# lucidrains/audiolm-pytorch

Hardware: AMD Instinct MI355X
Metric: audio-tokens/sec fwd+bwd, CoarseTransformer d=1024 seq=2048 (higher is better)
Workload: dtype bf16

## Files before the change

### audiolm-pytorch_amd/csrc/gemm.hip

```cpp
#include <algorithm>
#include <cstdlib>
#include <type_traits>

#include "common.hpp"
#include "../../include/audiolm_hip.h"

#ifndef ALM_GEMM_AUX_A
#define ALM_GEMM_AUX_A 0
#endif
#ifndef ALM_GEMM_AUX_B
#define ALM_GEMM_AUX_B 0
#endif

namespace {

constexpr int BK = 64;
constexpr unsigned OOB = 0x80000000u;

typedef __attribute__((address_space(3))) void lds_void;

struct GemmParams {
    const bf16_t* A;
    const bf16_t* B;
    void* C;
// ... 60 lines not shown
                        if (OUT_F32) {
                            const int ch = c0 / 4;
                            *reinterpret_cast<float4*>(slab + lr * ROWB + ((ch ^ (lr & (NCH - 1))) << 4)) = make_float4(v[0], v[1], v[2], v[3]);
                        } else {
                            const int ch = c0 / 8;
                            *reinterpret_cast<uint2*>(slab + lr * ROWB + ((ch ^ (lr & (NCH - 1))) << 4) + lh * 8) =
                                make_uint2(pack_bf2(v[0], v[1]), pack_bf2(v[2], v[3]));
                        }
                    }
                constexpr int LPR = NCH;
                constexpr int RPI = 64 / LPR;
#pragma unroll
                for (int it = 0; it < 32 / RPI; ++it) {
                    const int row = it * RPI + lane / LPR, ch = lane % LPR;
                    const uint4 val = *reinterpret_cast<const uint4*>(slab + row * ROWB + ((ch ^ (row & (NCH - 1))) << 4));
                    const int gm = mrow0 + row, gn = ncol0 + ch * (16 / ES);
#if defined(ALM_GEMM_WHATIF_NOSTORE)
                    if (gm < p.M && gn < p.N && val.x == 0x7fc12345u) *reinterpret_cast<uint4*>(Cb + ((long long)gm * p.ldc + gn) * ES) = val;
#else
                    if (gm < p.M && gn < p.N) {
                        uint4* dst = reinterpret_cast<uint4*>(Cb + ((long long)gm * p.ldc + gn) * ES);
                        typedef unsigned int u32x4 __attribute__((ext_vector_type(4)));
                        if (p.nt_store) __builtin_nontemporal_store(u32x4{val.x, val.y, val.z, val.w}, reinterpret_cast<u32x4*>(dst)); else *dst = val;
                    }
#endif
                }
            }
            return;
        }
    }
    const long long coff = coff0;
    const bool vec_ok = OUT_F32 ? ((p.ldc & 3) == 0 && (coff & 3) == 0 && ((uintptr_t)p.C & 15) == 0)
                                : ((p.ldc & 3) == 0 && (coff & 3) == 0 && ((uintptr_t)p.C & 7) == 0);
#pragma unroll
    for (int i = 0; i < TM; ++i) {
        const int gm = m0 + wr * (BM / WM) + i * 32 + lr;
        if (gm >= p.M) continue;
#pragma unroll
        for (int j = 0; j < TNB; ++j) {
#pragma unroll
            for (int g = 0; g < 4; ++g) {
                const int gn = n0 + wc * (BN / WN) + j * 32 + 8 * g + 4 * lh;
                if (gn >= p.N) continue;
                float v[4];
#pragma unroll
                for (int c = 0; c < 4; ++c) {
                    v[c] = acc[i][j][4 * g + c] * p.alpha;
                    if (p.bias && gn + c < p.N) v[c] += p.bias[gn + c];
                }
                const long long idx = coff + (long long)gm * p.ldc + gn;
                if (OUT_F32) {
                    float* C = reinterpret_cast<float*>(p.C) + idx;
                    if (vec_ok && gn + 3 < p.N) {
                        float4 o = make_float4(v[0], v[1], v[2], v[3]);
                        if (p.accumulate) { const float4 w = *reinterpret_cast<const float4*>(C); o.x += w.x; o.y += w.y; o.z += w.z; o.w += w.w; }
                        *reinterpret_cast<float4*>(C) = o;
                    } else {
#pragma unroll
                        for (int c = 0; c < 4; ++c)
                            if (gn + c < p.N) C[c] = p.accumulate ? C[c] + v[c] : v[c];
                    }
                } else {
                    bf16_t* C = reinterpret_cast<bf16_t*>(p.C) + idx;
                    if (vec_ok && gn + 3 < p.N) {
                        if (p.accumulate) {
                            const uint2 w = *reinterpret_cast<const uint2*>(C);
                            v[0] += __uint_as_float(w.x << 16); v[1] += __uint_as_float(w.x & 0xffff0000u);
                            v[2] += __uint_as_float(w.y << 16); v[3] += __uint_as_float(w.y & 0xffff0000u);
                        }
                        *reinterpret_cast<uint2*>(C) = make_uint2(pack_bf2(v[0], v[1]), pack_bf2(v[2], v[3]));
                    } else {
#pragma unroll
                        for (int c = 0; c < 4; ++c)
                            if (gn + c < p.N) C[c] = f2bf(p.accumulate ? bf2f(C[c]) + v[c] : v[c]);
                    }
                }
            }
        }
    }
}

template <int N>
__device__ __forceinline__ void wait_vmcnt() {
    static_assert(N == 0 || N == 8 || N == 16, "add the literal");
    if constexpr (N == 0) asm volatile("s_waitcnt vmcnt(0)" ::: "memory");
    else if constexpr (N == 8) asm volatile("s_waitcnt vmcnt(8)" ::: "memory");
    else asm volatile("s_waitcnt vmcnt(16)" ::: "memory");
}

template <int BM, int BN, int WM, int WN, bool TNMODE, bool OUT_F32, int NS = 2>
__device__ __forceinline__ void gemm_body(const GemmParams& p, const int bx, const int by, const int bz) {
    extern __shared__ __attribute__((aligned(1024))) unsigned char smem[];
    constexpr int NW = WM * WN;
    constexpr int A_BYTES = BM * BK * 2, B_BYTES = BN * BK * 2, STAGE = A_BYTES + B_BYTES;
    constexpr int TM = BM / WM / 32, TNB = BN / WN / 32;
    constexpr int NIA = BM / 8 / NW, NIB = BN / 8 / NW;
    static_assert(NIA >= 1 && NIB >= 1 && (BM / 8) % NW == 0 && (BN / 8) % NW == 0, "tile / wave shape");

    const int tiles_m = (p.M + BM - 1) / BM, tiles_n = (p.N + BN - 1) / BN;
    int tm, tn, zb, zs;
    if (p.raster >= 1) {
        const int L = bx, xcd = L & 7, j = L >> 3;
        const bool m_major = tiles_m >= tiles_n;
        const int tmaj = m_major ? tiles_m : tiles_n, Q = m_major ? tiles_n : tiles_m;
        const int P = p.plimit > 0 ? p.plimit : tmaj * (p.nbt > 0 ? p.nbt : p.nb2);
        const int PL = (P + 7) / 8;
        zs = j / (PL * Q);
        const int rem = j % (PL * Q);
        const int panel = p.raster == 2 ? xcd * PL + rem / Q : (rem / Q) * 8 + xcd;
        const int minor = rem % Q;
        if (panel >= P || zs >= p.nsl) return;
        zb = panel / tmaj;
        const int tmajor = panel % tmaj;
        tm = m_major ? tmajor : minor;
        tn = m_major ? minor : tmajor;
    } else {
        const int nwg = tiles_m * tiles_n;
        const int bid = xcd_remap(bx, nwg);
        const int tt = grouped_tile(bid, tiles_m, tiles_n, p.group_m);
        tm = tt & 0xffff;
        tn = tt >> 16;
        zb = by;
        zs = bz;
    }
    const int m0 = tm * BM, n0 = tn * BN;

    const int z1 = zb / p.nb2, z2 = zb % p.nb2;
    int kbeg = 0, Krem = p.K;
    const long long zoffA = z1 * p.sA1 + z2 * p.sA2, zoffB = z1 * p.sB1 + z2 * p.sB2;
    if (p.ksplit > 0) {
        kbeg = zs * p.ksplit;
        Krem = min(p.K - kbeg, p.ksplit);
    }

    const int t = threadIdx.x;
    const int lane = t & 63;
    const int wave = __builtin_amdgcn_readfirstlane(t >> 6);
    const int wr = wave / WN, wc = wave % WN;
    const int lr = lane & 31, lh = lane >> 5;

    const bf16_t* Ab;
    const bf16_t* Bb;
    long long extA, extB;
    if (!TNMODE) {
        Ab = p.A + zoffA + (long long)m0 * p.lda + kbeg;
        Bb = p.B + zoffB + (long long)n0 * p.ldb + kbeg;
        extA = ((long long)(min(p.M - m0, BM) - 1) * p.lda + Krem) * 2;
        extB = ((long long)(min(p.N - n0, BN) - 1) * p.ldb + Krem) * 2;
    } else {
        Ab = p.A + zoffA + (long long)kbeg * p.lda + m0;
        Bb = p.B + zoffB + (long long)kbeg * p.ldb + n0;
        extA = ((long long)(Krem - 1) * p.lda + ((min(p.M - m0, BM) + 7) & ~7)) * 2;
        extB = ((long long)(Krem - 1) * p.ldb + ((min(p.N - n0, BN) + 7) & ~7)) * 2;
    }
    const auto rsA = __builtin_amdgcn_make_buffer_rsrc(const_cast<bf16_t*>(Ab), 0, (int)min(extA, 0x7fffffffLL), 0x00020000);
    const auto rsB = __builtin_amdgcn_make_buffer_rsrc(const_cast<bf16_t*>(Bb), 0, (int)min(extB, 0x7fffffffLL), 0x00020000);

    unsigned offA[NIA], offB[NIB];
    int kcA[NIA], kcB[NIB];
    if (!TNMODE) {
#pragma unroll
        for (int j = 0; j < NIA; ++j) {
            const int row = (j * NW + wave) * 8 + (lane >> 3);
            const int c = (lane & 7) ^ ((row >> 1) & 7);
            offA[j] = (unsigned)(row * p.lda * 2 + c * 16);
            kcA[j] = c * 8;
        }
#pragma unroll
// ... 367 lines not shown
    __builtin_amdgcn_s_barrier();

    if constexpr (INL) {
        typedef unsigned int u32x4 __attribute__((ext_vector_type(4)));
        constexpr int SLAB_BYTES = BM * BN * 4, NCHUNK = TM * TNB * 4;
        const int S = p.inl_slices;
        const int tile_lin = zb * (tiles_m * tiles_n) + tm * tiles_n + tn;
        unsigned char* const slab0 = reinterpret_cast<unsigned char*>(p.inl_ws) + (long long)tile_lin * S * SLAB_BYTES;
        {
            const auto rs = __builtin_amdgcn_make_buffer_rsrc(slab0 + (long long)zs * SLAB_BYTES, 0, SLAB_BYTES, 0x00020000);
#pragma unroll
            for (int i = 0; i < TM; ++i)
#pragma unroll
                for (int j = 0; j < TNB; ++j)
#pragma unroll
                    for (int g = 0; g < 4; ++g) {
                        const u32x4 v = {__float_as_uint(acc[i][j][4 * g]), __float_as_uint(acc[i][j][4 * g + 1]), __float_as_uint(acc[i][j][4 * g + 2]),
                                         __float_as_uint(acc[i][j][4 * g + 3])};
                        __builtin_amdgcn_raw_buffer_store_b128(v, rs, t * 16, ((i * TNB + j) * 4 + g) * 8192, 16);
                    }
        }
        asm volatile("s_waitcnt vmcnt(0)" ::: "memory");
        __syncthreads();
        unsigned* const flag = reinterpret_cast<unsigned*>(smem + 163840 - 16);
        if (t == 0) {
            const unsigned old = __hip_atomic_fetch_add(p.inl_cnt + tile_lin, 1u, __ATOMIC_RELAXED, __HIP_MEMORY_SCOPE_AGENT);
            const unsigned last = old == (unsigned)(S - 1);
            if (last) __hip_atomic_store(p.inl_cnt + tile_lin, 0u, __ATOMIC_RELAXED, __HIP_MEMORY_SCOPE_AGENT);
            *flag = last;
        }
        __syncthreads();
        if (*flag == 0) return;
        auto add_slab = [&](int sl, auto first_c) {
            constexpr bool FIRST = decltype(first_c)::value;
            const auto rs = __builtin_amdgcn_make_buffer_rsrc(slab0 + (long long)sl * SLAB_BYTES, 0, SLAB_BYTES, 0x00020000);
#pragma unroll
            for (int cb = 0; cb < NCHUNK; cb += 4) {
                u32x4 v[4];
#pragma unroll
                for (int c = 0; c < 4; ++c) v[c] = __builtin_amdgcn_raw_buffer_load_b128(rs, t * 16, (cb + c) * 8192, 16);
#pragma unroll
                for (int c = 0; c < 4; ++c)
#pragma unroll
                    for (int e = 0; e < 4; ++e) {
                        const int ai = (cb + c) / (4 * TNB), aj = ((cb + c) / 4) % TNB, ar = 4 * ((cb + c) % 4) + e;
                        acc[ai][aj][ar] = FIRST ? __uint_as_float(v[c][e]) : acc[ai][aj][ar] + __uint_as_float(v[c][e]);
                    }
            }
        };
        if (S == 2) {
            add_slab(1 - zs, std::false_type{});
        } else {
            add_slab(0, std::true_type{});
#pragma unroll 1
            for (int sl = 1; sl < S; ++sl) add_slab(sl, std::false_type{});
        }
    }

    const long long coff0 = z1 * p.sC1 + z2 * p.sC2 + (p.ksplit > 0 ? zs * p.sCk : 0);
    GPROBE_T(5);
    gemm_epilogue<BM, BN, WM, WN, TM, TNB, OUT_F32>(p, acc, smem, coff0, m0, n0, wave, wr, wc, lane, lr, lh);
    GPROBE_T(6);
    GPROBE_FLUSH((bx + gridDim.x * (by + gridDim.y * bz)) * 8 + wave);
}


template <bool TNMODE, bool OUT_F32>
__global__ __launch_bounds__(512) void gemm_stag_kernel(GemmParams p) {
    gemm_stag_body<TNMODE, OUT_F32>(p, blockIdx.x, blockIdx.y, blockIdx.z);
}

template <bool OUT_F32>
__global__ __launch_bounds__(512) void gemm_stag_inl_kernel(GemmParams p) {
    gemm_stag_body<false, OUT_F32, true>(p, blockIdx.x, blockIdx.y, blockIdx.z);
}

template <bool TNMODE, bool OUT_F32>
__global__ __launch_bounds__(512) void gemm_stag_group2_kernel(GemmParams p0, GemmParams p1, int tiles0) {
    const bool second = (int)blockIdx.x >= tiles0;
    const GemmParams& p = second ? p1 : p0;
    gemm_stag_body<TNMODE, OUT_F32>(p, second ? (int)blockIdx.x - tiles0 : (int)blockIdx.x, 0, 0);
}

template <bool TNMODE, bool OUT_F32>
__global__ __launch_bounds__(256) void gemm_w4_kernel(GemmParams p) {
    extern __shared__ __attribute__((aligned(1024))) unsigned char smem[];
    GPROBE_DECL
    constexpr int BM = 256, BN = 256, WM = 2, WN = 2, NW = 4, TM = 4, TNB = 4;
    constexpr int A_BYTES = BM * BK * 2, B_BYTES = BN * BK * 2, STAGE = A_BYTES + B_BYTES;
    constexpr int NIA = BM / 8 / NW, NIB = BN / 8 / NW;
    static_assert(NIA + NIB == 16, "the counted waits below assume 16 pieces per wave and stage");

    const int tiles_m = (p.M + BM - 1) / BM, tiles_n = (p.N + BN - 1) / BN;
    int tm, tn, zb, zs;
    if (p.raster >= 1) {
        const int L = blockIdx.x, xcd = L & 7, j = L >> 3;
        const bool m_major = tiles_m >= tiles_n;
        const int tmaj = m_major ? tiles_m : tiles_n, Q = m_major ? tiles_n : tiles_m;
        const int P = p.plimit > 0 ? p.plimit : tmaj * (p.nbt > 0 ? p.nbt : p.nb2);
        const int PL = (P + 7) / 8;
        zs = j / (PL * Q);
        const int rem = j % (PL * Q);
        const int panel = p.raster == 2 ? xcd * PL + rem / Q : (rem / Q) * 8 + xcd;
        const int minor = rem % Q;
        if (panel >= P || zs >= p.nsl) return;
        zb = panel / tmaj;
        const int tmajor = panel % tmaj;
        tm = m_major ? tmajor : minor;
        tn = m_major ? minor : tmajor;
    } else {
        const int nwg = tiles_m * tiles_n;
        const int bid = xcd_remap(blockIdx.x, nwg);
        const int tt = grouped_tile(bid, tiles_m, tiles_n, p.group_m);
        tm = tt & 0xffff;
        tn = tt >> 16;
        zb = blockIdx.y;
        zs = blockIdx.z;
    }
    const int m0 = tm * BM, n0 = tn * BN;
    const int z1 = zb / p.nb2, z2 = zb % p.nb2;
    int kbeg = 0, Krem = p.K;
    const long long zoffA = z1 * p.sA1 + z2 * p.sA2, zoffB = z1 * p.sB1 + z2 * p.sB2;
    if (p.ksplit > 0) {
        kbeg = zs * p.ksplit;
        Krem = min(p.K - kbeg, p.ksplit);
    }

    const int t = threadIdx.x;
    const int lane = t & 63;
    const int wave = __builtin_amdgcn_readfirstlane(t >> 6);
    const int wr = wave / WN, wc = wave % WN;
    const int lr = lane & 31, lh = lane >> 5;

    const bf16_t* Ab;
    const bf16_t* Bb;
    long long extA, extB;
    if (!TNMODE) {
        Ab = p.A + zoffA + (long long)m0 * p.lda + kbeg;
        Bb = p.B + zoffB + (long long)n0 * p.ldb + kbeg;
        extA = ((long long)(min(p.M - m0, BM) - 1) * p.lda + Krem) * 2;
        extB = ((long long)(min(p.N - n0, BN) - 1) * p.ldb + Krem) * 2;
    } else {
        Ab = p.A + zoffA + (long long)kbeg * p.lda + m0;
        Bb = p.B + zoffB + (long long)kbeg * p.ldb + n0;
        extA = ((long long)(Krem - 1) * p.lda + ((min(p.M - m0, BM) + 7) & ~7)) * 2;
        extB = ((long long)(Krem - 1) * p.ldb + ((min(p.N - n0, BN) + 7) & ~7)) * 2;
    }
    const auto rsA = __builtin_amdgcn_make_buffer_rsrc(const_cast<bf16_t*>(Ab), 0, (int)min(extA, 0x7fffffffLL), 0x00020000);
    const auto rsB = __builtin_amdgcn_make_buffer_rsrc(const_cast<bf16_t*>(Bb), 0, (int)min(extB, 0x7fffffffLL), 0x00020000);

    unsigned offA[NIA], offB[NIB];
    int kcA[NIA], kcB[NIB];
    if (!TNMODE) {
#pragma unroll
        for (int j = 0; j < NIA; ++j) {
            const int row = (j * NW + wave) * 8 + (lane >> 3);
            const int c = (lane & 7) ^ ((row >> 1) & 7);
            offA[j] = (unsigned)(row * p.lda * 2 + c * 16);
            kcA[j] = c * 8;
        }
#pragma unroll
        for (int j = 0; j < NIB; ++j) {
            const int row = (j * NW + wave) * 8 + (lane >> 3);
            const int c = (lane & 7) ^ ((row >> 1) & 7);
            offB[j] = (unsigned)(row * p.ldb * 2 + c * 16);
            kcB[j] = c * 8;
// ... 348 lines not shown
        }
        const uint4 pk = make_uint4(pack_bf2(e[0], e[1]), pack_bf2(e[2], e[3]), pack_bf2(e[4], e[5]), pack_bf2(e[6], e[7]));
        tile[i][cg * 4 + 0] = pk.x; tile[i][cg * 4 + 1] = pk.y; tile[i][cg * 4 + 2] = pk.z; tile[i][cg * 4 + 3] = pk.w;
        if (dst && r < q.rows_pad && c < q.cols_pad) *reinterpret_cast<uint4*>(dst + (long long)r * q.ld_dst + c) = pk;
    }
    if (!dstT) return;
    __syncthreads();
#pragma unroll
    for (int it = 0; it < 2; ++it) {
        const int w = it * 256 + t;
        const int rg = w & 7, cp = w >> 3;
        uint32_t a[8];
#pragma unroll
        for (int jj = 0; jj < 8; ++jj) a[jj] = tile[rg * 8 + jj][cp];
        const uint4 lo = make_uint4((a[0] & 0xffffu) | (a[1] << 16), (a[2] & 0xffffu) | (a[3] << 16), (a[4] & 0xffffu) | (a[5] << 16), (a[6] & 0xffffu) | (a[7] << 16));
        const uint4 hi = make_uint4((a[0] >> 16) | (a[1] & 0xffff0000u), (a[2] >> 16) | (a[3] & 0xffff0000u), (a[4] >> 16) | (a[5] & 0xffff0000u),
                                    (a[6] >> 16) | (a[7] & 0xffff0000u));
        const int oc = c0 + 2 * cp, orow = r0 + 8 * rg;
        if (orow < q.rows_pad) {
            if (oc < q.cols_pad) *reinterpret_cast<uint4*>(dstT + (long long)oc * q.ld_dstT + orow) = lo;
            if (oc + 1 < q.cols_pad) *reinterpret_cast<uint4*>(dstT + (long long)(oc + 1) * q.ld_dstT + orow) = hi;
        }
    }
}

template <int BM, int BN, int WM, int WN, bool TNMODE, bool OUT_F32>
int launch_cfg(const GemmParams& p, int ny, int nz, hipStream_t st) {
    constexpr int smem = 2 * (BM + BN) * BK * 2;
    static bool attr_done = false;
    auto kfn = gemm_kernel<BM, BN, WM, WN, TNMODE, OUT_F32>;
    if (!attr_done) {
        hipError_t e = hipFuncSetAttribute(reinterpret_cast<const void*>(kfn), hipFuncAttributeMaxDynamicSharedMemorySize, smem);
        if (e != hipSuccess) return (int)e;
        attr_done = true;
    }
    const int tiles_m = (p.M + BM - 1) / BM, tiles_n = (p.N + BN - 1) / BN;
    if (p.raster >= 1) {
        const int tmaj = tiles_m >= tiles_n ? tiles_m : tiles_n, Q = tiles_m >= tiles_n ? tiles_n : tiles_m;
        const int PL = ((p.plimit > 0 ? p.plimit : tmaj * ny) + 7) / 8;
        hipLaunchKernelGGL(kfn, dim3(8 * PL * Q * nz), dim3(WM * WN * 64), smem, st, p);
        return 0;
    }
    hipLaunchKernelGGL(kfn, dim3(tiles_m * tiles_n, ny, nz), dim3(WM * WN * 64), smem, st, p);
    return 0;
}

template <bool OUT_F32>
int launch_ring(const GemmParams& p, int ny, int nz, hipStream_t st) {
    constexpr int smem = 4 * (128 + 128) * BK * 2;
    static bool attr_done = false;
    auto kfn = gemm_ring_kernel<128, 128, 2, 2, false, OUT_F32, 4>;
    if (!attr_done) {
        hipError_t e = hipFuncSetAttribute(reinterpret_cast<const void*>(kfn), hipFuncAttributeMaxDynamicSharedMemorySize, smem);
        if (e != hipSuccess) return (int)e;
        attr_done = true;
    }
    hipLaunchKernelGGL(kfn, dim3(((p.M + 127) / 128) * ((p.N + 127) / 128), ny, nz), dim3(256), smem, st, p);
    return 0;
}

template <bool TNMODE, bool OUT_F32>
int launch_stag(const GemmParams& p, int ny, int nz, hipStream_t st) {
    constexpr int smem = 163840;
    static bool attr_done = false;
    auto kfn = gemm_stag_kernel<TNMODE, OUT_F32>;
    if (!attr_done) {
        hipError_t e = hipFuncSetAttribute(reinterpret_cast<const void*>(kfn), hipFuncAttributeMaxDynamicSharedMemorySize, smem);
        if (e != hipSuccess) return (int)e;
        attr_done = true;
    }
    const int tiles_m = (p.M + 255) / 256, tiles_n = (p.N + 255) / 256;
    if (p.raster >= 1) {
        const int tmaj = tiles_m >= tiles_n ? tiles_m : tiles_n, Q = tiles_m >= tiles_n ? tiles_n : tiles_m;
        const int PL = ((p.plimit > 0 ? p.plimit : tmaj * ny) + 7) / 8;
        hipLaunchKernelGGL(kfn, dim3(8 * PL * Q * nz), dim3(512), smem, st, p);
        return 0;
    }
    hipLaunchKernelGGL(kfn, dim3(tiles_m * tiles_n, ny, nz), dim3(512), smem, st, p);
    return 0;
}


template <bool OUT_F32>
int launch_stag_inl(const GemmParams& p, int ny, hipStream_t st) {
    constexpr int smem = 163840;
    static bool attr_done = false;
    auto kfn = gemm_stag_inl_kernel<OUT_F32>;
    if (!attr_done) {
        hipError_t e = hipFuncSetAttribute(reinterpret_cast<const void*>(kfn), hipFuncAttributeMaxDynamicSharedMemorySize, smem);
        if (e != hipSuccess) return (int)e;
        attr_done = true;
    }
    const int tiles_m = (p.M + 255) / 256, tiles_n = (p.N + 255) / 256;
    hipLaunchKernelGGL(kfn, dim3(tiles_m * tiles_n, ny, p.inl_slices), dim3(512), smem, st, p);
    return 0;
}

template <bool TNMODE, bool OUT_F32>
int launch_w4(const GemmParams& p, int ny, int nz, hipStream_t st) {
    constexpr int smem = 131072;
    static bool attr_done = false;
    auto kfn = gemm_w4_kernel<TNMODE, OUT_F32>;
    if (!attr_done) {
        hipError_t e = hipFuncSetAttribute(reinterpret_cast<const void*>(kfn), hipFuncAttributeMaxDynamicSharedMemorySize, smem);
        if (e != hipSuccess) return (int)e;
        attr_done = true;
    }
    const int tiles_m = (p.M + 255) / 256, tiles_n = (p.N + 255) / 256;
    if (p.raster >= 1) {
        const int tmaj = tiles_m >= tiles_n ? tiles_m : tiles_n, Q = tiles_m >= tiles_n ? tiles_n : tiles_m;
        const int PL = ((p.plimit > 0 ? p.plimit : tmaj * ny) + 7) / 8;
        hipLaunchKernelGGL(kfn, dim3(8 * PL * Q * nz), dim3(256), smem, st, p);
        return 0;
    }
    hipLaunchKernelGGL(kfn, dim3(tiles_m * tiles_n, ny, nz), dim3(256), smem, st, p);
    return 0;
}

int pick_tile(int M, int N, int ny, int tile, bool tn) {
    if (tile == 1 || tile == 2 || tile == 11 || tile == 13 || tile == 14 || tile == 15 || tile == 16 || tile == 17) return tile;
    if (tile != 0) return -1;
    if (M < 256 || N < 256) return 1;
    const long long t256 = (long long)((M + 255) / 256) * ((N + 255) / 256) * ny;
    if (t256 < 192) return 1;
    if (!tn) {
        static const double c320 = [] { const char* e = getenv("ALM_GEMM_T320_COST"); return e ? atoi(e) / 100.0 : 1.22; }();
        const long long t384 = (long long)((M + 383) / 384) * ((N + 255) / 256) * ny;
        const long long t320 = (long long)((M + 319) / 320) * ((N + 255) / 256) * ny;
        const double c13 = (double)((t256 + 255) / 256), c11 = (double)((t384 + 255) / 256) * 1.41;
        const double c17 = c320 > 0. ? (double)((t320 + 255) / 256) * c320 : 1e30;
        if (c17 < c13 && c17 < c11) return 17;
        if (c11 < c13) return 11;
    }
    return 13;
}

int pick_group(const GemmParams& p, int tl) {
    static const int env_g = [] { const char* e = getenv("ALM_GEMM_GROUP_M"); return e ? atoi(e) : 0; }();
    if (env_g != 0) return env_g;
    (void)p; (void)tl;
    return 8;
}

template <bool TNMODE>
int launch_gemm(const GemmParams& p0, int ny, int nz, int out_f32, int tile, hipStream_t st, bool hook = true, bool only256 = false) {
    static const int big_tile = [] { const char* e = getenv("ALM_GEMM_BIG_TILE"); return e ? atoi(e) : 0; }();
    static const int nt_store = [] { const char* e = getenv("ALM_GEMM_NT_STORE"); return e ? atoi(e) : 0; }();
    GemmParams p = p0;
    int tl = pick_tile(p.M, p.N, ny * nz, tile, TNMODE);
    if (tl < 0) return ALM_ERR_UNSUPPORTED;
    p.group_m = pick_group(p, tl);
    p.nt_store = (nt_store == 1 || (nt_store == 2 && !out_f32)) ? 1 : 0;
    if (hook && tl != 1 && (big_tile == 2 || big_tile == 13 || big_tile == 14 || (big_tile == 11 && !only256))) tl = big_tile;
    static const int w4_mink = [] { const char* e = getenv("ALM_GEMM_W4_MINK"); return e ? atoi(e) : 0; }();
    if (hook && w4_mink > 0 && tl == 13 && tile == 0 && (p.ksplit > 0 ? p.ksplit : p.K) >= w4_mink) tl = 14;
    static const int w4_tn_mink = [] { const char* e = getenv("ALM_GEMM_W4_TN_MINK"); return e ? atoi(e) : 8192; }();
    if (TNMODE && hook && w4_tn_mink > 0 && tl == 13 && (p.ksplit > 0 ? p.ksplit : p.K) >= w4_tn_mink) tl = 14;
    if (tl == 14) return out_f32 ? launch_w4<TNMODE, true>(p, ny, nz, st) : launch_w4<TNMODE, false>(p, ny, nz, st);
    if (tl == 13) return out_f32 ? launch_stag<TNMODE, true>(p, ny, nz, st) : launch_stag<TNMODE, false>(p, ny, nz, st);
    static const int mid_tile = [] { const char* e = getenv("ALM_GEMM_MID_TILE"); return e ? atoi(e) : 0; }();
    if (!TNMODE && hook && mid_tile && tl == 1 && tile == 0 && p.ksplit == 0 && p.M >= 256 && p.N >= 512 &&
        (long long)((p.M + 255) / 256) * ((p.N + 127) / 128) * ny >= 192) tl = 15;
    static const int ring_on = [] { const char* e = getenv("ALM_GEMM_RING"); return e ? atoi(e) : 1; }();
    if (!TNMODE && hook && ring_on && tl == 1 && tile == 0 && p.ksplit == 0 && p.raster == 0 && p.K >= 256 &&
        (long long)((p.M + 127) / 128) * ((p.N + 127) / 128) * ny * nz <= 256) tl = 16;
    if (tl == 16) { if (TNMODE || p.raster != 0) return ALM_ERR_UNSUPPORTED; return out_f32 ? launch_ring<true>(p, ny, nz, st) : launch_ring<false>(p, ny, nz, st); }
    if (tl == 15) return out_f32 ? launch_cfg<256, 128, 4, 2, TNMODE, true>(p, ny, nz, st) : launch_cfg<256, 128, 4, 2, TNMODE, false>(p, ny, nz, st);
    if (tl == 11) return out_f32 ? launch_cfg<384, 256, 2, 4, TNMODE, true>(p, ny, nz, st) : launch_cfg<384, 256, 2, 4, TNMODE, false>(p, ny, nz, st);
    if (tl == 17) { if (TNMODE) return ALM_ERR_UNSUPPORTED; return out_f32 ? launch_cfg<320, 256, 2, 4, false, true>(p, ny, nz, st) : launch_cfg<320, 256, 2, 4, false, false>(p, ny, nz, st); }
    if (tl == 2) return out_f32 ? launch_cfg<256, 256, 2, 4, TNMODE, true>(p, ny, nz, st) : launch_cfg<256, 256, 2, 4, TNMODE, false>(p, ny, nz, st);
    return out_f32 ? launch_cfg<128, 128, 2, 2, TNMODE, true>(p, ny, nz, st) : launch_cfg<128, 128, 2, 2, TNMODE, false>(p, ny, nz, st);
}

bool view_too_big(long long rows, long long ld) { return rows * ld * 2 >= 0x7fffffffLL; }

constexpr long long INL_CNT_BYTES = 4096, INL_SLAB_BYTES = 256 * 256 * 4;
struct NtPlan { int tile, slices; };

NtPlan nt_plan(int M, int N, int K, int nb) {
    static const int mode = [] { const char* e = getenv("ALM_GEMM_NT_INL"); return e ? atoi(e) : 1; }();
    const int base = pick_tile(M, N, nb, 0, false);
    if (mode == 0 || base != 1 || M < 256 || N < 256) return NtPlan{base, 1};
    const long long t256 = (long long)((M + 255) / 256) * ((N + 255) / 256) * nb;
    const long long t128 = (long long)((M + 127) / 128) * ((N + 127) / 128) * nb;
    if (t256 > 128) return NtPlan{base, 1};
    const int ksteps = (K + BK - 1) / BK;
    double best_t = t128 <= 256 ? ksteps * 0.72 + 4.5 : (double)((t128 + 511) / 512) * (ksteps * 1.31 + 4.5);
    NtPlan best{base, 1};
    for (int S = 2; S <= 8; ++S) {
        const long long W = t256 * S;
        if (W > 256) break;
        const int kc = (ksteps + S - 1) / S;
        if (kc < 4) break;
        if ((ksteps + kc - 1) / kc != S) continue;
        const double t = kc * (1.15 + 0.0033 * W) + 7.0 + (8.0 + 0.04 * W) + 2.6 * (S == 2 ? 1 : S);
        if (mode >= 2 ? (S == mode || best.slices == 1) : t < best_t) { best_t = t; best = NtPlan{13, S}; }
    }
    return best;
}

int nt_launch_ws(const GemmParams& p0, int ny, int out_f32, int force_slices, void* ws, long long ws_bytes, hipStream_t st) {
    NtPlan pl = nt_plan(p0.M, p0.N, p0.K, ny);
    if (force_slices > 0) {
        const long long t256 = (long long)((p0.M + 255) / 256) * ((p0.N + 255) / 256) * ny;
        if (p0.M < 256 || p0.N < 256 || t256 > 1024) return ALM_ERR_UNSUPPORTED;
        pl = NtPlan{13, force_slices};
    }
    if (force_slices == 0 && (pl.tile != 13 || pl.slices < 2)) return launch_gemm<false>(p0, ny, 1, out_f32, 0, st);
    const long long tiles = (long long)((p0.M + 255) / 256) * ((p0.N + 255) / 256) * ny;
    if (pl.slices == 1) return launch_gemm<false>(p0, ny, 1, out_f32, 13, st, false);
    const long long need = INL_CNT_BYTES + tiles * pl.slices * INL_SLAB_BYTES;
    if (!ws || ws_bytes < need || ((uintptr_t)ws & 15)) {
        if (force_slices > 0) return ALM_ERR_BAD_ARG;
        return launch_gemm<false>(p0, ny, 1, out_f32, 0, st);
    }
    GemmParams p = p0;
    const int ksteps = (p.K + BK - 1) / BK;
    p.ksplit = (ksteps + pl.slices - 1) / pl.slices * BK;
    p.sCk = 0;
    p.inl_slices = (p.K + p.ksplit - 1) / p.ksplit;
    if (p.inl_slices < 2) return launch_gemm<false>(p0, ny, 1, out_f32, 13, st, false);
    p.inl_cnt = reinterpret_cast<unsigned*>(ws);
    p.inl_ws = reinterpret_cast<float*>(reinterpret_cast<unsigned char*>(ws) + INL_CNT_BYTES);
    p.group_m = pick_group(p, 13);
    return out_f32 ? launch_stag_inl<true>(p, ny, st) : launch_stag_inl<false>(p, ny, st);
}

struct SplitPlan { int tile, slices; };

int pick_raster(int M, int N, int nb, int tile) {
    const int bm = tile >= 2 ? 256 : 128;
    const int tmm = (M + bm - 1) / bm, tnn = (N + bm - 1) / bm;
    const int P = (tmm >= tnn ? tmm : tnn) * nb;
    return (P % 8 == 0 || P >= 20) ? 1 : 0;
}
SplitPlan splitk_plan(int M, int N, int K, int nb) {
    SplitPlan best{1, 1};
    double best_t = 1e30;
    for (int tile = 1; tile <= 2; ++tile) {
        if (tile == 2 && (M < 256 || N < 256)) continue;
// ... 408 lines not shown
```

Measured before the change: 1.405 million.

## Add 8-wave 256x256 GEMM kernel with phased LDS reads and staged prefetch

Adds a new 512-thread 256x256 GEMM kernel for NN-mode problems. It splits each K-tile into half-tile quadrants and interleaves ds_read, buffer_load_lds prefetch for the next tiles and MFMA groups, using counted vmcnt waits and barriers to keep the matrix cores fed. When enough tiles exist and no raster or k-split is set, it becomes the default in place of the staggered 256 kernel. The risk is that the hand-tuned waits and barrier choreography stall or race, and that OOB handling in the tail tiles stays correct.

```diff
diff --git a/audiolm-pytorch_amd/csrc/gemm.hip b/audiolm-pytorch_amd/csrc/gemm.hip
--- a/audiolm-pytorch_amd/csrc/gemm.hip
+++ b/audiolm-pytorch_amd/csrc/gemm.hip
@@ -166,8 +166,11 @@
 
 template <int N>
 __device__ __forceinline__ void wait_vmcnt() {
-    static_assert(N == 0 || N == 8 || N == 16, "add the literal");
+    static_assert(N == 0 || N == 2 || N == 4 || N == 6 || N == 8 || N == 16, "add the literal");
     if constexpr (N == 0) asm volatile("s_waitcnt vmcnt(0)" ::: "memory");
+    else if constexpr (N == 2) asm volatile("s_waitcnt vmcnt(2)" ::: "memory");
+    else if constexpr (N == 4) asm volatile("s_waitcnt vmcnt(4)" ::: "memory");
+    else if constexpr (N == 6) asm volatile("s_waitcnt vmcnt(6)" ::: "memory");
     else if constexpr (N == 8) asm volatile("s_waitcnt vmcnt(8)" ::: "memory");
     else asm volatile("s_waitcnt vmcnt(16)" ::: "memory");
 }
@@ -701,6 +704,179 @@
     gemm_stag_body<TNMODE, OUT_F32>(p, second ? (int)blockIdx.x - tiles0 : (int)blockIdx.x, 0, 0);
 }
 
+template <int OFF>
+__device__ __forceinline__ void ph8_read_b(bf16x8 (&b)[4], const unsigned (&ad)[4]) {
+    asm volatile("ds_read_b128 %0, %1 offset:%2" : "=v"(b[0]) : "v"(ad[0]), "n"(OFF) : "memory");
+    asm volatile("ds_read_b128 %0, %1 offset:%2" : "=v"(b[1]) : "v"(ad[1]), "n"(OFF) : "memory");
+    asm volatile("ds_read_b128 %0, %1 offset:%2" : "=v"(b[2]) : "v"(ad[2]), "n"(OFF) : "memory");
+    asm volatile("ds_read_b128 %0, %1 offset:%2" : "=v"(b[3]) : "v"(ad[3]), "n"(OFF) : "memory");
+}
+template <int OFF>
+__device__ __forceinline__ void ph8_read_a(bf16x8 (&a)[2][4], const unsigned (&ad)[4]) {
+    asm volatile("ds_read_b128 %0, %1 offset:%2" : "=v"(a[0][0]) : "v"(ad[0]), "n"(OFF) : "memory");
+    asm volatile("ds_read_b128 %0, %1 offset:%2" : "=v"(a[1][0]) : "v"(ad[0]), "n"(OFF + 4096) : "memory");
+    asm volatile("ds_read_b128 %0, %1 offset:%2" : "=v"(a[0][1]) : "v"(ad[1]), "n"(OFF) : "memory");
+    asm volatile("ds_read_b128 %0, %1 offset:%2" : "=v"(a[1][1]) : "v"(ad[1]), "n"(OFF + 4096) : "memory");
+    asm volatile("ds_read_b128 %0, %1 offset:%2" : "=v"(a[0][2]) : "v"(ad[2]), "n"(OFF) : "memory");
+    asm volatile("ds_read_b128 %0, %1 offset:%2" : "=v"(a[1][2]) : "v"(ad[2]), "n"(OFF + 4096) : "memory");
+    asm volatile("ds_read_b128 %0, %1 offset:%2" : "=v"(a[0][3]) : "v"(ad[3]), "n"(OFF) : "memory");
+    asm volatile("ds_read_b128 %0, %1 offset:%2" : "=v"(a[1][3]) : "v"(ad[3]), "n"(OFF + 4096) : "memory");
+}
+
+template <bool OUT_F32>
+__global__ __launch_bounds__(512) void gemm_ph8_kernel(GemmParams p) {
+    extern __shared__ __attribute__((aligned(1024))) unsigned char smem[];
+    constexpr int BM = 256, BN = 256, WM = 2, WN = 4, TM = 4, TNB = 2;
+    constexpr int HALF = 128 * BK * 2;
+    constexpr int B_BASE = 4 * HALF;
+    static_assert(B_BASE + 4 * HALF == 131072 && 3 * HALF + 4096 < 65536, "LDS map / ds_read offset field");
+
+    const int tiles_m = (p.M + BM - 1) / BM, tiles_n = (p.N + BN - 1) / BN;
+    const int bid = xcd_remap(blockIdx.x, tiles_m * tiles_n);
+    const int tt = grouped_tile(bid, tiles_m, tiles_n, p.group_m);
+    const int m0 = (tt & 0xffff) * BM, n0 = (tt >> 16) * BN;
+    const int zb = blockIdx.y;
+    const int z1 = zb / p.nb2, z2 = zb % p.nb2;
+    const int Krem = p.K;
+
+    const int t = threadIdx.x;
+    const int lane = t & 63;
+    const int wave = __builtin_amdgcn_readfirstlane(t >> 6);
+    const int wr = wave / WN, wc = wave % WN;
+    const int lr = lane & 31, lh = lane >> 5;
+
+    const bf16_t* Ab = p.A + z1 * p.sA1 + z2 * p.sA2 + (long long)m0 * p.lda;
+    const bf16_t* Bb = p.B + z1 * p.sB1 + z2 * p.sB2 + (long long)n0 * p.ldb;
+    const long long extA = ((long long)(min(p.M - m0, BM) - 1) * p.lda + Krem) * 2;
+    const long long extB = ((long long)(min(p.N - n0, BN) - 1) * p.ldb + Krem) * 2;
+    const auto rsA = __builtin_amdgcn_make_buffer_rsrc(const_cast<bf16_t*>(Ab), 0, (int)min(extA, 0x7fffffffLL), 0x00020000);
+    const auto rsB = __builtin_amdgcn_make_buffer_rsrc(const_cast<bf16_t*>(Bb), 0, (int)min(extB, 0x7fffffffLL), 0x00020000);
+
+    const int rl0 = wave * 8 + (lane >> 3);
+    const int cs = (lane & 7) ^ ((rl0 >> 1) & 7);
+    const int kc = cs * 8;
+    unsigned offA[2][2], offB[2][2];
+#pragma unroll
+    for (int h = 0; h < 2; ++h)
+#pragma unroll
+        for (int i = 0; i < 2; ++i) {
+            const int rl = rl0 + 64 * i;
+            const int rowa = (rl >> 6) * 128 + h * 64 + (rl & 63), rowb = (rl >> 5) * 64 + h * 32 + (rl & 31);
+            offA[h][i] = (unsigned)(rowa * p.lda * 2 + cs * 16);
+            offB[h][i] = (unsigned)(rowb * p.ldb * 2 + cs * 16);
+        }
+    auto stage_a = [&](int kt, auto hc, auto bc) {
+        constexpr int H = decltype(hc)::value, BUF = decltype(bc)::value;
+        const int kleft = Krem - kt * BK;
+#pragma unroll
+        for (int i = 0; i < 2; ++i) {
+            const unsigned vo = (kc < kleft) ? offA[H][i] : OOB;
+            __builtin_amdgcn_raw_ptr_buffer_load_lds(rsA, (lds_void*)(smem + (BUF * 2 + H) * HALF + (wave + 8 * i) * 1024), 16, vo, kt * (BK * 2), 0, ALM_GEMM_AUX_A);
+        }
+    };
+    auto stage_b = [&](int kt, auto hc, auto bc) {
+        constexpr int H = decltype(hc)::value, BUF = decltype(bc)::value;
+        const int kleft = Krem - kt * BK;
+#pragma unroll
+        for (int i = 0; i < 2; ++i) {
+            const unsigned vo = (kc < kleft) ? offB[H][i] : OOB;
+            __builtin_amdgcn_raw_ptr_buffer_load_lds(rsB, (lds_void*)(smem + B_BASE + (BUF * 2 + H) * HALF + (wave + 8 * i) * 1024), 16, vo, kt * (BK * 2), 0, ALM_GEMM_AUX_B);
+        }
+    };
+
+    const unsigned lds0 = (unsigned)reinterpret_cast<uintptr_t>((lds_void*)smem);
+    const unsigned sw = (unsigned)((lr >> 1) & 7);
+    unsigned adA[4], adB[4];
+#pragma unroll
+    for (int ks = 0; ks < 4; ++ks) {
+        const unsigned co = (((unsigned)(ks * 2 + lh)) ^ sw) << 4;
+        adA[ks] = lds0 + (unsigned)((wr * 64 + lr) * 128) + co;
+        adB[ks] = lds0 + (unsigned)(B_BASE + (wc * 32 + lr) * 128) + co;
+    }
+
+    f32x16 acc[TM][TNB];
+#pragma unroll
+    for (int i = 0; i < TM; ++i)
+#pragma unroll
+        for (int j = 0; j < TNB; ++j)
+#pragma unroll
+            for (int r = 0; r < 16; ++r) acc[i][j][r] = 0.f;
+
+    using I0 = std::integral_constant<int, 0>;
+    using I1 = std::integral_constant<int, 1>;
+    using I2 = std::integral_constant<int, 2>;
+    auto open = [&]() {
+        __builtin_amdgcn_sched_barrier(0);
+        __builtin_amdgcn_s_barrier();
+        asm volatile("s_waitcnt lgkmcnt(0)" ::: "memory");
+        __builtin_amdgcn_sched_barrier(0);
+    };
+    auto mfma8 = [&](auto ic, auto jc, const bf16x8 (&a)[2][4], const bf16x8 (&b)[4]) {
+        constexpr int I = decltype(ic)::value, J = decltype(jc)::value;
+        __builtin_amdgcn_s_setprio(1);
+#pragma unroll
+        for (int ks = 0; ks < 4; ++ks)
+#pragma unroll
+            for (int i2 = 0; i2 < 2; ++i2) acc[I + i2][J] = __builtin_amdgcn_mfma_f32_32x32x16_bf16(b[ks], a[i2][ks], acc[I + i2][J], 0, 0, 0);
+        __builtin_amdgcn_s_setprio(0);
+        __builtin_amdgcn_sched_barrier(0);
+        __builtin_amdgcn_s_barrier();
+        __builtin_amdgcn_sched_barrier(0);
+    };
+    const int nk = (Krem + BK - 1) / BK;
+    auto ktile = [&](auto bufc, int T) {
+        constexpr int BUF = decltype(bufc)::value;
+        using BC = std::integral_constant<int, BUF>;
+        using BO = std::integral_constant<int, BUF ^ 1>;
+        const bool more1 = T + 1 < nk, more2 = T + 2 < nk;
+        bf16x8 al[2][4], ah[2][4], bl[4], bh[4];
+        ph8_read_b<(BUF * 2 + 0) * HALF>(bl, adB);
+        __builtin_amdgcn_sched_barrier(0);
+        ph8_read_a<(BUF * 2 + 0) * HALF>(al, adA);
+        if (more1) stage_a(T + 1, I1{}, BO{});
+        else wait_vmcnt<2>();
+        asm volatile("s_waitcnt lgkmcnt(8)" ::: "memory");
+        open();
+        mfma8(I0{}, I0{}, al, bl);
+        ph8_read_b<(BUF * 2 + 1) * HALF>(bh, adB);
+        if (more2) stage_b(T + 2, I0{}, BC{});
+        else if (!more1) wait_vmcnt<0>();
+        open();
+        mfma8(I0{}, I1{}, al, bh);
+        ph8_read_a<(BUF * 2 + 1) * HALF>(ah, adA);
+        if (more2) stage_a(T + 2, I0{}, BC{});
+        open();
+        mfma8(I2{}, I1{}, ah, bh);
+        if (more2) { stage_b(T + 2, I1{}, BC{}); wait_vmcnt<6>(); }
+        else if (more1) wait_vmcnt<4>();
+        open();
+        mfma8(I2{}, I0{}, ah, bl);
+    };
+
+    stage_b(0, I0{}, I0{}); stage_a(0, I0{}, I0{}); stage_b(0, I1{}, I0{}); stage_a(0, I1{}, I0{});
+    if (nk == 1) {
+        wait_vmcnt<4>();
+    } else {
+        stage_b(1, I0{}, I1{}); stage_a(1, I0{}, I1{}); stage_b(1, I1{}, I1{});
+        wait_vmcnt<6>();
+    }
+    __builtin_amdgcn_s_barrier();
+    if (wr == 1) __builtin_amdgcn_s_barrier();
+    int T = 0;
+#pragma unroll 1
+    for (; T + 1 < nk; T += 2) {
+        ktile(I0{}, T);
+        ktile(I1{}, T + 1);
+    }
+    if (T < nk) ktile(I0{}, T);
+    if (wr == 0) __builtin_amdgcn_s_barrier();
+
+    constexpr int ES = OUT_F32 ? 4 : 2;
+    static_assert(WM * WN * 32 * (32 * TNB * ES) <= B_BASE + 4 * HALF, "epilogue slab");
+    const long long coff0 = z1 * p.sC1 + z2 * p.sC2;
+    gemm_epilogue<BM, BN, WM, WN, TM, TNB, OUT_F32>(p, acc, smem, coff0, m0, n0, wave, wr, wc, lane, lr, lh);
+}
+
 template <bool TNMODE, bool OUT_F32>
 __global__ __launch_bounds__(256) void gemm_w4_kernel(GemmParams p) {
     extern __shared__ __attribute__((aligned(1024))) unsigned char smem[];
@@ -1215,6 +1391,21 @@
 
 
 template <bool OUT_F32>
+int launch_ph8(const GemmParams& p, int ny, hipStream_t st) {
+    constexpr int smem = 131072;
+    static bool attr_done = false;
+    auto kfn = gemm_ph8_kernel<OUT_F32>;
+    if (!attr_done) {
+        hipError_t e = hipFuncSetAttribute(reinterpret_cast<const void*>(kfn), hipFuncAttributeMaxDynamicSharedMemorySize, smem);
+        if (e != hipSuccess) return (int)e;
+        attr_done = true;
+    }
+    const int tiles_m = (p.M + 255) / 256, tiles_n = (p.N + 255) / 256;
+    hipLaunchKernelGGL(kfn, dim3(tiles_m * tiles_n, ny, 1), dim3(512), smem, st, p);
+    return 0;
+}
+
+template <bool OUT_F32>
 int launch_stag_inl(const GemmParams& p, int ny, hipStream_t st) {
     constexpr int smem = 163840;
     static bool attr_done = false;
@@ -1251,7 +1442,7 @@
 }
 
 int pick_tile(int M, int N, int ny, int tile, bool tn) {
-    if (tile == 1 || tile == 2 || tile == 11 || tile == 13 || tile == 14 || tile == 15 || tile == 16 || tile == 17) return tile;
+    if (tile == 1 || tile == 2 || tile == 11 || tile == 13 || tile == 14 || tile == 15 || tile == 16 || tile == 17 || tile == 18) return tile;
     if (tile != 0) return -1;
     if (M < 256 || N < 256) return 1;
     const long long t256 = (long long)((M + 255) / 256) * ((N + 255) / 256) * ny;
@@ -1273,6 +1464,11 @@
     if (env_g != 0) return env_g;
     (void)p; (void)tl;
     return 8;
+}
+
+bool ph8_rule(long long tiles, int ksteps) {
+    static const int on = [] { const char* e = getenv("ALM_GEMM_PH8"); return e ? atoi(e) : 1; }();
+    return on != 0 && tiles >= 192 && ksteps >= 1;
 }
 
 template <bool TNMODE>
@@ -1289,6 +1485,12 @@
     if (hook && w4_mink > 0 && tl == 13 && tile == 0 && (p.ksplit > 0 ? p.ksplit : p.K) >= w4_mink) tl = 14;
     static const int w4_tn_mink = [] { const char* e = getenv("ALM_GEMM_W4_TN_MINK"); return e ? atoi(e) : 8192; }();
     if (TNMODE && hook && w4_tn_mink > 0 && tl == 13 && (p.ksplit > 0 ? p.ksplit : p.K) >= w4_tn_mink) tl = 14;
+    if constexpr (!TNMODE) {
+        if (tl == 18 && (p.raster != 0 || p.ksplit > 0 || nz != 1)) return ALM_ERR_UNSUPPORTED;
+        if (hook && tile == 0 && tl == 13 && p.raster == 0 && p.ksplit == 0 && nz == 1 &&
+            (big_tile == 18 || (big_tile == 0 && ph8_rule((long long)((p.M + 255) / 256) * ((p.N + 255) / 256) * ny, (p.K + BK - 1) / BK)))) tl = 18;
+        if (tl == 18) return out_f32 ? launch_ph8<true>(p, ny, st) : launch_ph8<false>(p, ny, st);
+    } else if (tl == 18) return ALM_ERR_UNSUPPORTED;
     if (tl == 14) return out_f32 ? launch_w4<TNMODE, true>(p, ny, nz, st) : launch_w4<TNMODE, false>(p, ny, nz, st);
     if (tl == 13) return out_f32 ? launch_stag<TNMODE, true>(p, ny, nz, st) : launch_stag<TNMODE, false>(p, ny, nz, st);
     static const int mid_tile = [] { const char* e = getenv("ALM_GEMM_MID_TILE"); return e ? atoi(e) : 0; }();
```

Result: no change. 1.404 million (-0.1%).
